# martinber/noaa-apt

Hardware: AMD Instinct MI355X
Metric: Msamples/sec WAV->APT-line decode (higher is better)
Workload: dtype f32; 1 GPU; synthetic 48000 Hz APT recording, 600 s (28800000 samples) per GPU, profile=standard: resample 13/50 (959 taps) -> AM envelope -> 37-tap low-pass -> sync correlation + peak picker -> 1198 rows x 2080 px; parallelism=1 GPU(s), 16 independent recordings per GPU and step, no collectives, recordings_per_call=16, mode=strict, rows=1198, n_sync=1199, input_resident_in_hbm=True, distinct_inputs_round_robin=16

## Files before the change

noaa_apt_amd/csrc/apt_kernels.hpp:

```cpp
#pragma once

#include <hip/hip_runtime.h>

#include <cstdint>

namespace apt::gpu {

struct Result {
    int32_t status;
    int32_t reason;
    uint32_t n_rows;
    uint32_t n_sync;
    uint64_t work_len;
    uint64_t n_out;
};

struct ImageResult {
    int32_t status;
    int32_t reason;
    uint32_t height;
    uint32_t telemetry_row;
    float low, high;
    float telemetry_quality;
    int32_t channel_a, channel_b;
    uint32_t reserved;
    uint64_t n_px;
    float values_a[16], values_b[16];
};

struct GroupMax {
    float hi;
    float lo;
};

struct LaunchSwitches {
    int gather_iters = 1;
    bool words_dpp = true;
    bool orbit_lds = true;
    int orbit_threads = 0;
    int orbit_alg = 1;
    float gm_slack_scale = 1.f;
    int fused_lds_pad = 0;
};
LaunchSwitches read_launch_switches();

constexpr int kMaxCall = 32;
struct RecArgs {
    const void *x;
    uint64_t n;
    uint64_t w;
    float *rows;
    uint32_t rows_cap;
    uint32_t slot;
};
struct CallArgs {
    uint32_t count;
    uint32_t tiles_x;
    RecArgs rec[kMaxCall];
};
struct SlotPtrs {
    float *f;
    GroupMax *gm;
    const float *corr;
    uint64_t *words;
    uint64_t *nanw;
    uint32_t *slot_nt, *slot_cnt, *flags, *orbit_ws, *peaks;
    Result *res;
    uint32_t peaks_cap;
    uint32_t reserved;
};

void resample_generic(hipStream_t s, const float *x, uint64_t n, const float *coeff,
                      uint32_t ntaps, uint32_t l, uint32_t m, float *out, uint64_t w);
uint32_t f16taps_pairs_per_phase(uint32_t l, uint32_t ntaps);
float f16taps_pack(uint32_t l, const float *coeff, uint32_t ntaps, uint16_t *table);
void resample_f16taps(hipStream_t s, const float *x, uint64_t n, const uint16_t *table, uint32_t ntaps,
                      uint32_t l, uint32_t m, float unscale, float *out, uint64_t w);
void fir_decimate(hipStream_t s, const float *x, uint64_t n, const float *coeff, uint32_t ntaps,
                  uint32_t m, float *out, uint64_t n_out);
void demodulate(hipStream_t s, const float *x, uint64_t n, float cosphi2, float sinphi, float *out);
void correlate(hipStream_t s, const float *f, uint64_t n_corr, uint32_t pw, float *corr);
void terminals(hipStream_t s, const float *corr, uint64_t n_corr, uint32_t md, uint64_t *bits);
void orbit_walk(hipStream_t s, const uint64_t *bits, const float *corr, uint64_t n_corr, uint64_t work_len,
                uint32_t spr, uint32_t md, uint32_t *peaks, uint32_t peaks_cap, Result *res);
void gather_rows(hipStream_t s, const float *f, const uint32_t *peaks, Result *res,
                 uint32_t spr, uint32_t pw, bool raw, float *rows, uint32_t rows_cap);
void gather_rows_call(hipStream_t s, const CallArgs &call, const SlotPtrs *d_slots, uint32_t spr, uint32_t pw,
                      uint32_t max_rows_cap, const LaunchSwitches &sw = LaunchSwitches{});

void nosync_rows_call(hipStream_t s, const CallArgs &call, const SlotPtrs *d_slots, uint32_t spr, uint32_t m2, uint64_t max_w);

bool fused_supported(uint32_t l, uint32_t m, uint32_t t1, uint32_t t2, uint32_t pw);
uint32_t fused_group_size(uint32_t l);
bool fused_takes_pcm16(uint32_t l, uint32_t m);
uint32_t fused_tap_table_floats(uint32_t l, uint32_t m, uint32_t t1, int ch);
void fused_branch_taps(uint32_t l, uint32_t m, const float *coeff, uint32_t t1, int ch, float *hs, uint32_t t1_layout = 0);
uint32_t fused_pad_t1(uint32_t l, uint32_t m, uint32_t t1, uint32_t t2, uint32_t pw);
uint32_t fused_pad_t2(uint32_t l, uint32_t m, uint32_t t2, uint32_t pw);
uint32_t fused_phase_pad_t2(uint32_t t2, uint32_t pw);
int fused_chunk_of(uint32_t m, bool fast);
void fused_lowpass_pairs(const float *h2, uint32_t t2, float *h2p);
uint32_t fused_f16_table_dwords(uint32_t l, uint32_t m, uint32_t t1);
float fused_f16_branch_taps(uint32_t l, uint32_t m, const float *coeff, uint32_t t1, uint32_t *table);
bool fused_f16_supported(uint32_t l, uint32_t m, uint32_t t1, uint32_t t2, uint32_t pw);
float fused_gm_slack(uint32_t pw, float scale = 1.f);
bool fused_fast_supported(uint32_t l, uint32_t m, uint32_t t1, uint32_t t2, uint32_t pw);
struct TableGeom {
    uint32_t l, m;
    uint32_t jlim;
    uint32_t tpp;
    uint32_t xt;
    uint32_t off_x;
    uint32_t step_q, step_r;
    uint32_t jl_a, jl_b;
    uint32_t nthr, perm_off, nperm;
    uint32_t nq;
    uint32_t sq;
    uint32_t stream;
    uint32_t exact, perm_shift, cp_off, xd;
    uint32_t tt_off;
// ... 81 lines not shown
```

noaa_apt_amd/csrc/apt_kernels_generic.hip:

```cpp
#include "apt_kernels.hpp"
#include "apt_envelope.hpp"

#include <hip/hip_runtime.h>

#include <cstdlib>

#include <cmath>
#include <cstring>
#include <map>
#include <mutex>
#include <tuple>

#pragma clang fp contract(off)

namespace apt::gpu {

namespace {

constexpr int kBlock = 256;

inline unsigned grid_for(uint64_t n, unsigned block, unsigned cap = 256u * 32u)
{
    uint64_t g = (n + block - 1) / block;
    if (g > cap) g = cap;
// ... 380 lines not shown
    hipLaunchKernelGGL(k_resample_generic, dim3(grid_for(w, kBlock)), dim3(kBlock), 0, s, x, n,
                       coeff, jlim, l, m, out, w);
}

uint32_t f16taps_pairs_per_phase(uint32_t l, uint32_t ntaps) { return ((ntaps + l - 1) / l + 1) / 2; }

float f16taps_pack(uint32_t l, const float *coeff, uint32_t ntaps, uint16_t *table)
{
    const uint32_t jlim = 2 * ((ntaps - 1) / 2) + 1;
    const uint32_t tp2 = f16taps_pairs_per_phase(l, ntaps);
    float mx = 0.f;
    for (uint32_t j = 0; j < jlim; ++j) mx = fmaxf(mx, fabsf(coeff[j]));
    int e = 0;
    if (mx > 0.f) (void)frexpf(mx, &e);
    const int sh = -e + 1;
    const float scale = ldexpf(1.f, sh);
    for (uint32_t p = 0; p < l; ++p)
        for (uint32_t i = 0; i < 2 * tp2; ++i) {
            const uint64_t j = p + static_cast<uint64_t>(i) * l;
            const _Float16 h = static_cast<_Float16>(j < jlim ? coeff[j] * scale : 0.f);
            uint16_t bits;
            __builtin_memcpy(&bits, &h, 2);
            table[(static_cast<size_t>(p) * tp2 * 2) + i] = bits;
        }
    return ldexpf(1.f, -sh);
}

void resample_f16taps(hipStream_t s, const float *x, uint64_t n, const uint16_t *table, uint32_t ntaps,
                      uint32_t l, uint32_t m, float unscale, float *out, uint64_t w)
{
    if (w == 0) return;
    hipLaunchKernelGGL(k_resample_f16taps, dim3(grid_for(w, kBlock)), dim3(kBlock), 0, s, x, n,
                       reinterpret_cast<const h2 *>(table), f16taps_pairs_per_phase(l, ntaps), l, m, unscale,
                       out, w);
}

void fir_decimate(hipStream_t s, const float *x, uint64_t , const float *coeff,
                  uint32_t ntaps, uint32_t m, float *out, uint64_t n_out)
{
    if (n_out == 0) return;
    hipLaunchKernelGGL(k_fir_decimate, dim3(grid_for(n_out, kBlock)), dim3(kBlock), 0, s, x, coeff,
                       ntaps, m, out, n_out);
}

void demodulate(hipStream_t s, const float *x, uint64_t n, float cosphi2, float sinphi, float *out)
{
    if (n == 0) return;
    hipLaunchKernelGGL(k_demodulate, dim3(grid_for(n, kBlock)), dim3(kBlock), 0, s, x, n, cosphi2,
                       sinphi, out);
}

void correlate(hipStream_t s, const float *f, uint64_t n_corr, uint32_t pw, float *corr)
{
    if (n_corr == 0) return;
    hipLaunchKernelGGL(k_correlate, dim3(grid_for(n_corr, kBlock)), dim3(kBlock), 0, s, f, n_corr,
                       pw, corr);
}

void terminals(hipStream_t s, const float *corr, uint64_t n_corr, uint32_t md, uint64_t *bits)
{
    if (n_corr == 0) return;
    const unsigned blocks = static_cast<unsigned>((n_corr + md - 1) / md);
    const size_t lds = static_cast<size_t>(2) * md * sizeof(float);
    if (lds > 48 * 1024)
        (void)hipFuncSetAttribute(reinterpret_cast<const void *>(k_terminals),
                                  hipFuncAttributeMaxDynamicSharedMemorySize,
                                  static_cast<int>(lds));
    hipLaunchKernelGGL(k_terminals, dim3(blocks), dim3(kTermThreads), lds, s, corr, n_corr, md,
                       bits);
}

void orbit_walk(hipStream_t s, const uint64_t *bits, const float *corr, uint64_t n_corr, uint64_t work_len,
                uint32_t spr, uint32_t md, uint32_t *peaks, uint32_t peaks_cap, Result *res)
{
    hipLaunchKernelGGL(k_orbit_walk, dim3(1), dim3(64), 0, s, bits, corr, n_corr, work_len, spr, md,
                       peaks, peaks_cap, res);
}

LaunchSwitches read_launch_switches()
{
    LaunchSwitches sw;
    if (const char *e = std::getenv("APTGPU_GATHER_ITERS")) sw.gather_iters = std::atoi(e);
    if (const char *e = std::getenv("APTGPU_WORDS_DPP")) sw.words_dpp = e[0] != '0';
    if (const char *e = std::getenv("APTGPU_ORBIT_LDS")) sw.orbit_lds = e[0] != '0';
    if (const char *e = std::getenv("APTGPU_ORBIT_THREADS")) sw.orbit_threads = std::atoi(e);
    if (const char *e = std::getenv("APTGPU_ORBIT_ALG")) sw.orbit_alg = e[0] == '0' ? 0 : 1;
    if (const char *e = std::getenv("APTGPU_GM_SLACK_SCALE")) {
        const float v = std::strtof(e, nullptr);
        if (v >= 1.f) sw.gm_slack_scale = v;
    }
    if (const char *e = std::getenv("APTGPU_FUSED_LDS_PAD")) sw.fused_lds_pad = std::max(0, std::atoi(e));
    return sw;
}

void gather_rows_call(hipStream_t s, const CallArgs &call, const SlotPtrs *d_slots, uint32_t spr, uint32_t pw,
                      uint32_t max_rows_cap, const LaunchSwitches &sw)
{
    if (call.count == 0) return;
    {
        const int iters = sw.gather_iters;
        bool aligned = true;
        for (uint32_t i = 0; i < call.count; ++i) aligned = aligned && (reinterpret_cast<uintptr_t>(call.rec[i].rows) & 15u) == 0;
        if (iters > 0 && spr / pw == 2080u && spr % pw == 0 && aligned && max_rows_cap > 0) {
            const uint64_t quads = static_cast<uint64_t>(max_rows_cap < 32768u ? max_rows_cap : 32768u) * 520u;
            const uint64_t per_wg = static_cast<uint64_t>(kBlock) * static_cast<uint64_t>(iters);
            const unsigned gx = static_cast<unsigned>((quads + per_wg - 1) / per_wg);
            hipLaunchKernelGGL(k_gather_rows_flat<520u>, dim3(gx ? gx : 1, call.count), dim3(kBlock), 0, s, call, d_slots, spr, pw);
            return;
        }
    }
    const unsigned rows_cap = max_rows_cap < 32768u ? max_rows_cap : 32768u;
    const unsigned gy = max_rows_cap == 0 ? 1u : (rows_cap + 7u) / 8u;
    const unsigned gx = (spr / pw + 4 * kBlock - 1) / (4 * kBlock);
    hipLaunchKernelGGL(k_gather_rows_call, dim3(gx ? gx : 1, gy, call.count), dim3(kBlock), 0, s, call, d_slots,
                       spr, pw);
}

void gather_rows(hipStream_t s, const float *f, const uint32_t *peaks, Result *res,
                 uint32_t spr, uint32_t pw, bool raw, float *rows, uint32_t rows_cap)
{
    const unsigned gy = rows_cap == 0 ? 1u : (rows_cap < 4096u ? rows_cap : 4096u);
    const unsigned gx = (spr / pw + 4 * kBlock - 1) / (4 * kBlock);
    hipLaunchKernelGGL(k_gather_rows, dim3(gx ? gx : 1, gy), dim3(kBlock), 0, s, f, peaks, res, spr,
                       pw, raw ? 1 : 0, rows, rows_cap);
}


__global__ void __launch_bounds__(256) k_verify_fast_divide(float c, float rc, uint32_t *bad)
{
    const uint32_t i = blockIdx.x * 256u + threadIdx.x;
    const float x = __uint_as_float(0x3F800000u + i);
    const float want = x / c;
    const float got = fast_divide(x, c, rc);
    if (__float_as_uint(want) != __float_as_uint(got)) atomicAdd(bad, 1u);
}

__global__ void __launch_bounds__(256) k_verify_fast_sqrt(uint32_t lo, uint32_t count, uint32_t *bad)
{
    const uint64_t base = (static_cast<uint64_t>(blockIdx.x) * 256u + threadIdx.x) * 64u;
    uint32_t b = 0;
    for (uint32_t i = 0; i < 64u; ++i) {
        const uint64_t idx = base + i;
        if (idx >= count) break;
        const float x = __uint_as_float(lo + static_cast<uint32_t>(idx));
        b += __float_as_uint(exact_sqrt_inrange(x)) != __float_as_uint(__builtin_sqrtf(x));
    }
    if (b) atomicAdd(bad, b);
}

static bool verify_fast_sqrt(int device, hipStream_t s, uint32_t *d_bad)
{
    static std::mutex mu;
    static std::map<int, bool> cache;
    std::lock_guard<std::mutex> lock(mu);
    if (auto it = cache.find(device); it != cache.end()) return it->second;
    constexpr uint32_t lo = 0x0F800000u, hi = 0x71800000u;
    constexpr uint32_t count = hi - lo + 1u, threads = (count + 63u) / 64u;
    uint32_t bad = 1;
    bool ok = hipMemsetAsync(d_bad, 0, sizeof(uint32_t), s) == hipSuccess;
    if (ok) {
        hipLaunchKernelGGL(k_verify_fast_sqrt, dim3((threads + 255u) / 256u), dim3(256), 0, s, lo, count, d_bad);
        ok = hipGetLastError() == hipSuccess &&
             hipMemcpyAsync(&bad, d_bad, sizeof(uint32_t), hipMemcpyDeviceToHost, s) == hipSuccess &&
             hipStreamSynchronize(s) == hipSuccess;
    }
    if (ok) cache[device] = bad == 0;
// ... 39 lines not shown
```

noaa_apt_amd/csrc/apt_kernels_sync.hip:

```cpp
#include "apt_kernels.hpp"
#include "apt_sync_corr.hpp"

#include <hip/hip_runtime.h>

#include <atomic>

#include <cstdlib>
#include <type_traits>

namespace apt::gpu {

namespace {

constexpr int GS = 52;
constexpr uint64_t kGroupMask = (1ull << GS) - 1;
constexpr float kNegInf = -__builtin_huge_valf();

__global__ void __launch_bounds__(256)
k_group_max(const float *__restrict__ corr, uint64_t n_corr, GroupMax *__restrict__ gm, uint32_t ng)
{
    const uint32_t g = blockIdx.x * blockDim.x + threadIdx.x;
    if (g >= ng) return;
    const uint64_t base = static_cast<uint64_t>(g) * GS;
    float mx = kNegInf;
    bool has_nan = false;
    for (int o = 0; o < GS; ++o) {
        const uint64_t i = base + o;
        if (i < n_corr) {
            float v = corr[i];
            if (i == 0 && !(v > 0.f)) v = 0.f;
            mx = fmaxf(mx, v);
            has_nan = has_nan || (v != v);
        }
    }
    gm[g] = has_nan ? GroupMax{-kNegInf, kNegInf} : GroupMax{mx, mx};
}

constexpr int kNodesThreads = 128;
constexpr int kNodesWaves = kNodesThreads / 64;
constexpr int kChunkGroups = 128;
constexpr int kSlotCap = 64;
static_assert(kNodesThreads == kChunkGroups, "one thread per own group");
constexpr uint32_t kNanStartTag = 0x80000000u;
constexpr uint32_t kPosMask = 0x7FFFFFFFu;

__host__ __device__ constexpr uint32_t nodes_window(uint32_t pw) { return (GS + 38u * pw - 1u + 3u) & ~3u; }

__device__ __forceinline__ float wave_prefix_max_dpp(float x)
{
    asm volatile("s_nop 1\n\tv_max_f32_dpp %0, %0, %0 row_shr:1 row_mask:0xf bank_mask:0xf\n\t"
                 "s_nop 1\n\tv_max_f32_dpp %0, %0, %0 row_shr:2 row_mask:0xf bank_mask:0xf\n\t"
                 "s_nop 1\n\tv_max_f32_dpp %0, %0, %0 row_shr:4 row_mask:0xf bank_mask:0xf\n\t"
                 "s_nop 1\n\tv_max_f32_dpp %0, %0, %0 row_shr:8 row_mask:0xf bank_mask:0xf\n\t"
                 "s_nop 1\n\tv_max_f32_dpp %0, %0, %0 row_bcast:15 row_mask:0xa bank_mask:0xf\n\t"
                 "s_nop 1\n\tv_max_f32_dpp %0, %0, %0 row_bcast:31 row_mask:0xc bank_mask:0xf\n\t"
                 "s_nop 1"
                 : "+v"(x));
    return x;
}
__device__ __forceinline__ float wave_suffix_max_excl_dpp(float x, int lane)
{
    float y = -__builtin_huge_valf();
    asm volatile("s_nop 1\n\tv_mov_b32_dpp %0, %1 wave_shl:1 row_mask:0xf bank_mask:0xf\n\t"
                 "s_nop 1\n\tv_max_f32_dpp %0, %0, %0 row_shl:1 row_mask:0xf bank_mask:0xf\n\t"
                 "s_nop 1\n\tv_max_f32_dpp %0, %0, %0 row_shl:2 row_mask:0xf bank_mask:0xf\n\t"
                 "s_nop 1\n\tv_max_f32_dpp %0, %0, %0 row_shl:4 row_mask:0xf bank_mask:0xf\n\t"
                 "s_nop 1\n\tv_max_f32_dpp %0, %0, %0 row_shl:8 row_mask:0xf bank_mask:0xf\n\t"
                 "s_nop 1"
                 : "+v"(y)
                 : "v"(x));
    const float r1 = __builtin_bit_cast(float, __builtin_amdgcn_readlane(__builtin_bit_cast(int, y), 16));
    const float r2 = __builtin_bit_cast(float, __builtin_amdgcn_readlane(__builtin_bit_cast(int, y), 32));
    const float r3 = __builtin_bit_cast(float, __builtin_amdgcn_readlane(__builtin_bit_cast(int, y), 48));
    const float m23 = fmaxf(r2, r3), m123 = fmaxf(r1, m23);
    const float tail = lane < 16 ? m123 : lane < 32 ? m23 : lane < 48 ? r3 : -__builtin_huge_valf();
    return fmaxf(y, tail);
}

__host__ __device__ constexpr uint32_t words_f32_ofs() { return kChunkGroups * 16u; }
__host__ __device__ constexpr uint32_t words_win_ofs(uint32_t r)
{
    return (words_f32_ofs() + (kChunkGroups + r + 1) * 16u + kChunkGroups * 4u + kChunkGroups * 2u + 15u) & ~15u;
}

template <int NL, int PWC>
__device__ __forceinline__ float nodes_eval_window(float *win, bool on, int lane, uint32_t pw, int fast)
{
    constexpr int NLR = NL > 0 ? NL : 1;
    float c = kNegInf;
    if (fast) {
        const uint32_t blen = GS + 36u * pw;
        if constexpr (NL > 0) {
            float bs[NLR];
#pragma unroll
            for (int t = 0; t < NL; ++t) {
                const uint32_t pq = lane + 64u * t;
                bs[t] = pq < blen ? sync_pulse_sum(pw, [&](uint32_t j) { return win[pq + j]; }) : 0.f;
            }
            __builtin_amdgcn_wave_barrier();
#pragma unroll
            for (int t = 0; t < NL; ++t) {
                const uint32_t pq = lane + 64u * t;
                if (pq < blen) win[pq] = bs[t];
            }
            __builtin_amdgcn_wave_barrier();
        } else {
            for (uint32_t p0 = 0; p0 < blen; p0 += 64) {
                const uint32_t pq = p0 + lane;
                const float bs = pq < blen ? sync_pulse_sum(pw, [&](uint32_t j) { return win[pq + j]; }) : 0.f;
                __builtin_amdgcn_wave_barrier();
                if (pq < blen) win[pq] = bs;
                __builtin_amdgcn_wave_barrier();
            }
        }
        if (on) c = sync_corr_from_pulses([&](int k) { return win[lane + k * 2 * pw]; });
    } else {
        if constexpr (PWC >= 4) {
            if (on) c = sync_corr_strict_rolled(pw, [&](uint32_t j) { return win[lane + j]; });
        } else {
            if (on) c = sync_corr_strict(pw, [&](uint32_t j) { return win[lane + j]; });
        }
    }
    return c;
}

template <int NL, int PWC, bool DPP>
__global__ void __launch_bounds__(kNodesThreads, 4)
k_sync_words(const CallArgs call, const SlotPtrs *__restrict__ slots, uint32_t pw_arg, uint32_t r_groups ,
             int fast, int use_corr)
{
    const uint32_t pw = PWC > 0 ? static_cast<uint32_t>(PWC) : pw_arg;
    const RecArgs rec = call.rec[blockIdx.y];
    const uint64_t w = rec.w;
    const uint64_t n_corr = w - 38ull * pw;
    const uint32_t ng = static_cast<uint32_t>((n_corr + GS - 1) / GS);
    if (blockIdx.x * static_cast<uint32_t>(kChunkGroups) >= ng) return;
    const SlotPtrs sp = slots[rec.slot];
    const GroupMax *__restrict__ gm = sp.gm;
    const float *__restrict__ corr = use_corr ? sp.corr : nullptr;
    const float *__restrict__ fsig = sp.f;
    uint32_t *__restrict__ flags = sp.flags;

    extern __shared__ uint64_t lds_nodes[];
    const int R = static_cast<int>(r_groups);
    const int N = kChunkGroups + R + 1;
    uint64_t *s_words = lds_nodes;
    uint64_t *s_nanw = s_words + kChunkGroups;
    float *s_hi = reinterpret_cast<float *>(reinterpret_cast<char *>(lds_nodes) + words_f32_ofs());
    float *s_lo = s_hi + N;
    float *s_ma = s_lo + N;
    float *s_mb = s_ma + N;
    float *s_wm = s_mb + N;
    uint16_t *s_cand = reinterpret_cast<uint16_t *>(s_wm + kChunkGroups);
    const uint32_t wlen = nodes_window(pw);
    float *s_win = reinterpret_cast<float *>(reinterpret_cast<char *>(lds_nodes) + words_win_ofs(r_groups));
    __shared__ uint32_t s_ncand;

    const int tid = threadIdx.x;
    const int lane = tid & 63;
    const int wave = tid >> 6;
    const int64_t g0 = static_cast<int64_t>(blockIdx.x) * kChunkGroups;
    const int64_t gw0 = g0;
    const uint64_t md = static_cast<uint64_t>(R) * GS;

    if (tid == 0) s_ncand = 0;
    if (blockIdx.x == 0 && tid == 0) {
        sp.res->status = -1;
        sp.res->reason = -1;
    }
    for (int q = tid; q < N; q += kNodesThreads) {
        const int64_t g = g0 + q;
        const GroupMax v = g < static_cast<int64_t>(ng) ? gm[g] : GroupMax{kNegInf, kNegInf};
        s_hi[q] = v.hi;
        s_lo[q] = v.lo;
        s_ma[q] = v.lo;
    }
    s_words[tid] = 0ull;
    s_nanw[tid] = 0ull;
    __syncthreads();

    {
        const int W = R - 1;
        float *a = s_ma, *bq = s_mb;
        int K = 1;
        for (; 2 * K <= W; K *= 2) {
            for (int q = tid; q < N; q += kNodesThreads) bq[q] = (q + K < N) ? fmaxf(a[q], a[q + K]) : a[q];
            __syncthreads();
            float *t = a; a = bq; bq = t;
        }
        const int q = tid;
        const int64_t g = g0 + q;
        const float wm = fmaxf(a[q + 1], a[q + 1 + W - K]);
        s_wm[q] = wm;
        if (g < static_cast<int64_t>(ng) && !(wm > s_hi[q])) s_cand[atomicAdd(&s_ncand, 1u)] = static_cast<uint16_t>(q);
        __syncthreads();
    }

    const uint32_t ncand = s_ncand;
    constexpr int kBatch = NL > 0 ? 4 : 1;
    constexpr int NLR = NL > 0 ? NL : 1;
    constexpr uint16_t kDeferred = 0x8000u;
    float *wa = s_win + static_cast<size_t>(wave) * wlen;
    const uint32_t wneed = GS + 38u * pw - 1u;
    auto eval_group = [&](uint64_t base, bool on) -> float {
        for (uint32_t t = lane; t < wlen; t += 64) {
            const uint64_t j = base + t;
            wa[t] = (t < wneed && j < w) ? fsig[j] : 0.f;
        }
        __builtin_amdgcn_wave_barrier();
        const float v = nodes_eval_window<NL, PWC>(wa, on, lane, pw, fast);
        __builtin_amdgcn_wave_barrier();
        return v;
    };
    auto settle = [&](auto exact_tag, int q, float cv, float c2v, bool in_v) -> bool {
        constexpr bool EXACT = decltype(exact_tag)::value;
        const uint64_t base = static_cast<uint64_t>(gw0 + q) * GS;
        const bool in2 = in_v && base + lane + md < n_corr;
        if (in_v && gw0 + q == 0 && lane == 0 && !(cv > 0.f)) cv = 0.f;
        const unsigned long long nanword = __ballot(in_v && cv != cv) & kGroupMask;
        if (cv != cv) cv = kNegInf;
        float sfx_ex;
        if constexpr (DPP) {
            sfx_ex = wave_suffix_max_excl_dpp(cv, lane);
        } else {
            float sfx = cv;
            for (int d = 1; d < 64; d <<= 1) {
                const float o = __shfl_down(sfx, d, 64);
                if (lane + d < 64) sfx = fmaxf(sfx, o);
            }
            sfx_ex = __shfl_down(sfx, 1, 64);
            if (lane == 63) sfx_ex = kNegInf;
        }
        float wm = s_wm[q];
        const bool open_lo = in_v && !(sfx_ex > cv) && !(wm > cv);
        if (__ballot(open_lo) != 0ull) {
            float wm_hi = kNegInf;
            for (int h = q + 1 + lane; h < q + R; h += 64) wm_hi = fmaxf(wm_hi, s_hi[h]);
            for (int d = 32; d >= 1; d >>= 1) wm_hi = fmaxf(wm_hi, __shfl_xor(wm_hi, d, 64));
            const bool open = open_lo && wm_hi > cv;
            if (__ballot(open) != 0ull) {
                if constexpr (!EXACT) {
                    return false;
                } else {
                    float thr = open ? cv : -kNegInf;
                    for (int d = 32; d >= 1; d >>= 1) thr = fminf(thr, __shfl_xor(thr, d, 64));
                    float ex = kNegInf;
#pragma unroll 1
                    for (int h0 = q + 1; h0 < q + R; h0 += 64) {
                        unsigned long long todo = __ballot(h0 + lane < q + R && s_hi[h0 + lane] > thr);
                        while (todo) {
                            const int h = h0 + __ffsll(static_cast<long long>(todo)) - 1;
                            todo &= todo - 1;
                            const int64_t gh = gw0 + h;
                            if (gh >= static_cast<int64_t>(ng)) break;
                            const uint64_t hb = static_cast<uint64_t>(gh) * GS;
                            const bool on = lane < GS && hb + lane < n_corr;
                            float v = kNegInf;
                            if (corr != nullptr) {
                                if (on) v = corr[hb + lane];
                            } else {
                                v = eval_group(hb, on);
                            }
                            if (v != v) v = kNegInf;
                            ex = fmaxf(ex, v);
                        }
                    }
                    for (int d = 32; d >= 1; d >>= 1) ex = fmaxf(ex, __shfl_xor(ex, d, 64));
                    if (open) wm = ex;
                    if (lane == 0) atomicAdd(&flags[7], 1u);
                }
            }
        }
        float wmax = fmaxf(sfx_ex, wm);
        const float gm_ahead = s_hi[q + R];
        if (corr == nullptr && __ballot(in2 && !(wmax > cv) && gm_ahead > cv) != 0ull) c2v = eval_group(base + md, in2);
        if (c2v != c2v) c2v = kNegInf;
        float pfx = c2v;
        if constexpr (DPP) {
            pfx = wave_prefix_max_dpp(pfx);
        } else {
            for (int d = 1; d < 64; d <<= 1) {
                const float o = __shfl_up(pfx, d, 64);
                if (lane >= d) pfx = fmaxf(pfx, o);
            }
        }
        wmax = fmaxf(wmax, pfx);
        const bool term = in_v && !(wmax > cv);
        const unsigned long long word = __ballot(term) & kGroupMask;
        if (lane == 0) {
            s_words[q] = word;
            s_nanw[q] = nanword;
        }
        __builtin_amdgcn_wave_barrier();
        return true;
    };
    bool any_deferred = false;
    for (uint32_t c0 = wave * kBatch; c0 < ncand; c0 += kBatch * kNodesWaves) {
        int qv[kBatch];
        float cv[kBatch], c2v[kBatch];
        bool inv[kBatch];
        float fa[kBatch][NLR];
#pragma unroll
        for (int e = 0; e < kBatch; ++e) {
            const uint32_t ci = c0 + e;
            qv[e] = (ci < ncand) ? s_cand[ci] : -1;
            const int64_t g = gw0 + (qv[e] < 0 ? 0 : qv[e]);
            const uint64_t i = static_cast<uint64_t>(g) * GS + lane;
            inv[e] = qv[e] >= 0 && lane < GS && i < n_corr;
            cv[e] = kNegInf;
            c2v[e] = kNegInf;
            if (corr != nullptr) {
                if (inv[e]) {
                    cv[e] = corr[i];
                    if (i + md < n_corr) c2v[e] = corr[i + md];
                }
            } else if constexpr (NL > 0) {
#pragma unroll
                for (int t = 0; t < NL; ++t) {
                    const uint64_t j = static_cast<uint64_t>(g) * GS + lane + 64u * t;
                    fa[e][t] = (qv[e] >= 0 && lane + 64u * t < wneed && j < w) ? fsig[j] : 0.f;
                }
            }
        }
#pragma unroll
        for (int e = 0; e < kBatch; ++e) {
            if (qv[e] < 0) continue;
            if (corr == nullptr) {
                if constexpr (NL > 0) {
#pragma unroll
                    for (int t = 0; t < NL; ++t)
                        if (lane + 64u * t < wlen) wa[lane + 64 * t] = fa[e][t];
                    __builtin_amdgcn_wave_barrier();
                    cv[e] = nodes_eval_window<NL, PWC>(wa, inv[e], lane, pw, fast);
                    __builtin_amdgcn_wave_barrier();
                } else {
                    cv[e] = eval_group(static_cast<uint64_t>(gw0 + qv[e]) * GS, inv[e]);
                }
            }
            if (!settle(std::false_type{}, qv[e], cv[e], c2v[e], inv[e])) {
                if (lane == 0) s_cand[c0 + e] = static_cast<uint16_t>(qv[e]) | kDeferred;
                any_deferred = true;
            }
        }
    }
    if (any_deferred) {
#pragma unroll 1
        for (uint32_t c0 = wave * kBatch; c0 < ncand; c0 += kBatch * kNodesWaves) {
#pragma unroll 1
            for (uint32_t ci = c0; ci < c0 + kBatch && ci < ncand; ++ci) {
                const uint16_t ent = s_cand[ci];
                if (!(ent & kDeferred)) continue;
                const int q = ent & (kDeferred - 1);
                const uint64_t base = static_cast<uint64_t>(gw0 + q) * GS;
                const bool in_v = lane < GS && base + lane < n_corr;
                float cv = kNegInf, c2v = kNegInf;
                if (corr != nullptr) {
                    if (in_v) {
                        cv = corr[base + lane];
                        if (base + lane + md < n_corr) c2v = corr[base + lane + md];
                    }
                } else {
                    cv = eval_group(base, in_v);
                }
                (void)settle(std::true_type{}, q, cv, c2v, in_v);
            }
        }
    }
    __syncthreads();

    {
        const int64_t g = g0 + tid;
        if (g < static_cast<int64_t>(ng)) {
            sp.words[g] = s_words[tid];
            sp.nanw[g] = s_nanw[tid];
        }
    }
}

__global__ void __launch_bounds__(kNodesThreads)
k_sync_slots(const CallArgs call, const SlotPtrs *__restrict__ slots, uint32_t pw, uint32_t r_groups ,
             uint32_t grid_groups )
{
    const RecArgs rec = call.rec[blockIdx.y];
    const uint64_t n_corr = rec.w - 38ull * pw;
    const uint32_t ng = static_cast<uint32_t>((n_corr + GS - 1) / GS);
    if (blockIdx.x * static_cast<uint32_t>(kChunkGroups) >= ng) return;
    const SlotPtrs sp = slots[rec.slot];
    const uint64_t *__restrict__ words = sp.words;
    const uint64_t *__restrict__ nanw = sp.nanw;
    uint32_t *__restrict__ slot_nt = sp.slot_nt;
    __shared__ uint32_t s_scan[kNodesWaves];
    const int tid = threadIdx.x;
    const int lane = tid & 63;
    const int wave = tid >> 6;
    const int64_t R = r_groups;
    const int64_t g = static_cast<int64_t>(blockIdx.x) * kChunkGroups + tid;
    auto word_at = [&](const uint64_t *p, int64_t gi) -> uint64_t {
        return (gi >= 0 && gi < static_cast<int64_t>(ng)) ? p[gi] : 0ull;
    };
    uint64_t nw = 0, ns = 0;
    if (g < static_cast<int64_t>(ng)) {
        const uint64_t wd = words[g];
        const uint64_t nb = nanw[g];
        const uint64_t prev_bit = word_at(words, g - 1) >> (GS - 1);
        const uint64_t heads = wd & ~(((wd << 1) | prev_bit) & kGroupMask);
        const uint64_t shifted = ((word_at(words, g - R) << 1) | (word_at(words, g - R - 1) >> (GS - 1))) & kGroupMask;
        const uint64_t shifted_nan = ((word_at(nanw, g - R) << 1) | (word_at(nanw, g - R - 1) >> (GS - 1))) & kGroupMask;
        const uint64_t on_grid = (g % grid_groups == 0) ? 1ull : 0ull;
        const uint64_t starts = shifted | shifted_nan | on_grid;
        nw = wd & (heads | starts);
        ns = nb & starts & ~wd;
    }
    const uint32_t cnt = static_cast<uint32_t>(__popcll(nw | ns));
    uint32_t inc = cnt;
    for (int d = 1; d < 64; d <<= 1) {
        const uint32_t o = __shfl_up(inc, d, 64);
        if (lane >= d) inc += o;
    }
    if (lane == 63) s_scan[wave] = inc;
    __syncthreads();
    uint32_t base = 0;
    for (int wv = 0; wv < wave; ++wv) base += s_scan[wv];
    uint32_t total = 0;
    for (int wv = 0; wv < kNodesWaves; ++wv) total += s_scan[wv];
    uint32_t ofs = base + inc - cnt;
    uint64_t bitsleft = nw | ns;
    while (bitsleft) {
        const int bpos = __ffsll(static_cast<long long>(bitsleft)) - 1;
        bitsleft &= bitsleft - 1;
        if (ofs < kSlotCap)
            slot_nt[static_cast<uint64_t>(blockIdx.x) * kSlotCap + ofs] =
                static_cast<uint32_t>(static_cast<uint64_t>(g) * GS + bpos) | (((ns >> bpos) & 1ull) ? kNanStartTag : 0u);
        ++ofs;
    }
    if (tid == 0) {
        sp.slot_cnt[blockIdx.x] = total;
        if (total > kSlotCap) atomicOr(&sp.flags[0], 1u);
    }
}

constexpr int kOrbitThreadsMax = 1024;
constexpr int kMaxLevels = 64;

struct OrbitGeom {
    uint64_t n_corr, work_len;
    uint32_t spr, md;
};

__device__ __forceinline__ uint64_t first_terminal52(const uint64_t *__restrict__ words,
                                                     uint64_t n_groups, uint64_t s)
{
    const int lane = threadIdx.x & 63;
    uint64_t g0 = s / GS;
    const uint32_t sh = static_cast<uint32_t>(s % GS);
    bool first = true;
    while (true) {
        const uint64_t gi = g0 + lane;
        uint64_t word = (gi < n_groups) ? words[gi] : 0ull;
        if (first && lane == 0) word &= (~0ull) << sh;
        const unsigned long long any = __ballot(word != 0ull);
        if (any) {
            const int src = __ffsll(static_cast<long long>(any)) - 1;
            const uint64_t pos = gi * GS + (__ffsll(static_cast<long long>(word)) - 1);
            return __shfl(pos, src, 64);
        }
        first = false;
        g0 += 64;
        if (g0 >= n_groups) return ~0ull;
    }
}

__device__ void orbit_walk52(const uint64_t *__restrict__ words, const uint64_t *__restrict__ nanw,
                             const OrbitGeom &gq, uint32_t *__restrict__ peaks, uint32_t peaks_cap,
                             Result *__restrict__ res)
{
    auto nan_at = [&](uint64_t s) -> bool { return (nanw[s / GS] >> (s % GS)) & 1ull; };
    const int lane = threadIdx.x & 63;
    const uint64_t n_groups = (gq.n_corr + GS - 1) / GS;
    const uint64_t spr = gq.spr, md = gq.md;
    uint64_t len = 1;
    uint64_t u = 0;
    if (gq.n_corr > 0) u = first_terminal52(words, n_groups, 0);
    if (lane == 0 && peaks_cap > 0) peaks[0] = static_cast<uint32_t>(u);
    uint64_t fit = (u + spr < gq.work_len) ? 1 : 0;
    uint64_t last_fit = fit;
    while (gq.n_corr > 0) {
        const uint64_t a = u + md + 1;
        const uint64_t b = (len + 1) * spr;
        const uint64_t s = a > b ? a : b;
        if (s >= gq.n_corr) break;
        const uint64_t c = s / spr;
        for (uint64_t q = len + lane; q + 1 < c; q += 64)
            if (q < peaks_cap) peaks[q] = static_cast<uint32_t>(s);
        if (s + spr < gq.work_len) fit += c - len - 1;
        u = nan_at(s) ? s : first_terminal52(words, n_groups, s);
        if (lane == 0 && c - 1 < peaks_cap) peaks[c - 1] = static_cast<uint32_t>(u);
        last_fit = (u + spr < gq.work_len) ? 1 : 0;
        fit += last_fit;
        len = c;
    }
// ... 614 lines not shown
    }
    unsigned long long fit_local = 0;
    for (uint32_t k = tid; !peaks_done && k < path_cap; k += NT) {
        const uint32_t v = gld(w_path + k);
        if (v == END) continue;
        uint32_t cell;
        const uint32_t sv = node_start(v, &cell);
        const uint32_t u = gld(w_u + v);
        const bool is_last = (k + 1 >= path_cap) || gld(w_path + k + 1) == END;
        if (k == 0) {
            if (peaks_cap > 0) peaks[0] = u;
            if (!is_last && u + spr < wl32) ++fit_local;
            if (is_last) s_plen = 1;
            continue;
        }
        uint32_t pcell;
        (void)node_start(gld(w_path + k - 1), &pcell);
        const uint32_t c_prev = (k - 1 == 0) ? 1u : pcell;
        const uint32_t c = cell;
        for (uint32_t qv = c_prev; qv + 1 < c; ++qv)
            if (qv < peaks_cap) peaks[qv] = sv;
        if (c - 1 < peaks_cap) peaks[c - 1] = u;
        if (sv + spr < wl32) fit_local += c - c_prev - 1;
        if (!is_last && u + spr < wl32) ++fit_local;
        if (is_last) s_plen = c;
    }
    if (!peaks_done) {
    {
        uint32_t f32v = static_cast<uint32_t>(fit_local);
        for (int d = 32; d >= 1; d >>= 1) f32v += __shfl_down(f32v, d, 64);
        if ((tid & 63) == 0 && f32v) atomicAdd(&s_fit, static_cast<unsigned long long>(f32v));
    }
    __syncthreads();
    }
    if (tid == 0) {
        const uint32_t len = s_plen;
        const bool few = len < 5;
        const uint64_t rows = s_fit;
        res->status = few ? 1 : 0;
        res->reason = few ? 2 : 0;
        res->n_sync = len;
        res->n_rows = few ? 0 : static_cast<uint32_t>(rows);
        res->work_len = gq.work_len;
        res->n_out = few ? 0 : rows * 2080u;
        flags[1] = 2u;
        flags[0] = 0u;
        flags[5] = 0u;
        flags[2] = nt_cap;
        flags[3] = n_nodes;
        flags[4] = all_done ? n_all : count;
        flags[6] = all_done ? 3u : direct ? 1u : (in_lds ? 2u : 0u);
        if (all_done) flags[12] = 0u;
        flags[11] = flags7;
        flags[7] = 0u;
    }
    stamp(2);
}

}

uint32_t sync_group_size() { return GS; }
uint32_t sync_chunk_groups() { return kChunkGroups; }
uint32_t sync_slot_cap() { return kSlotCap; }

void group_max(hipStream_t s, const float *corr, uint64_t n_corr, GroupMax *gm)
{
    const uint32_t ng = static_cast<uint32_t>((n_corr + GS - 1) / GS);
    if (ng == 0) return;
    hipLaunchKernelGGL(k_group_max, dim3((ng + 255) / 256), dim3(256), 0, s, corr, n_corr, gm, ng);
}

void sync_nodes(hipStream_t s, const CallArgs &call, const SlotPtrs *d_slots, uint64_t max_w, uint32_t pw,
                uint32_t spr, uint32_t md, bool fast, bool use_corr, const LaunchSwitches &sw)
{
    if (call.count == 0 || max_w <= 38ull * pw) return;
    const uint64_t n_corr = max_w - 38ull * pw;
    const uint32_t ng = static_cast<uint32_t>((n_corr + GS - 1) / GS);
    const uint32_t chunks = (ng + kChunkGroups - 1) / kChunkGroups;
    const uint32_t r = md / GS;
    const size_t lds = words_win_ofs(r) + static_cast<size_t>(kNodesWaves) * nodes_window(pw) * sizeof(float);
    const dim3 grid(chunks, call.count);
    const uint32_t wneed = GS + 38u * pw - 1u;
    const bool dpp = sw.words_dpp;
#define APT_WORDS_LAUNCH(NL, PWC)                                                                                       \
    do {                                                                                                                \
        if (dpp)                                                                                                        \
            hipLaunchKernelGGL((k_sync_words<NL, PWC, true>), grid, dim3(kNodesThreads), lds, s, call, d_slots, pw, r,  \
                               fast ? 1 : 0, use_corr ? 1 : 0);                                                         \
        else                                                                                                            \
            hipLaunchKernelGGL((k_sync_words<NL, PWC, false>), grid, dim3(kNodesThreads), lds, s, call, d_slots, pw, r, \
                               fast ? 1 : 0, use_corr ? 1 : 0);                                                         \
    } while (0)
    if (pw == 3) APT_WORDS_LAUNCH(3, 3);
    else if (pw == 4) APT_WORDS_LAUNCH(4, 4);
    else if (pw == 5) APT_WORDS_LAUNCH(4, 5);
    else if (wneed <= 192) APT_WORDS_LAUNCH(3, 0);
    else if (wneed <= 256) APT_WORDS_LAUNCH(4, 0);
    else APT_WORDS_LAUNCH(0, 0);
#undef APT_WORDS_LAUNCH
    hipLaunchKernelGGL(k_sync_slots, grid, dim3(kNodesThreads), 0, s, call, d_slots, pw, r, spr / GS);
}

uint32_t sync_nt_cap(uint64_t w)
{
    const uint64_t ng = (w + GS - 1) / GS;
    const uint64_t chunks = (ng + kChunkGroups - 1) / kChunkGroups;
    return static_cast<uint32_t>(chunks * kSlotCap);
}

size_t sync_orbit_ws_words(uint64_t w, uint32_t spr)
{
    const uint64_t nt_cap = sync_nt_cap(w);
    const uint64_t kc = (spr ? w / spr : 0) + 2;
    const uint64_t node_cap = 1 + kc + nt_cap + 1;
    return 4 * node_cap + (node_cap / 32 + 1) + (kc + 2) + (kc + 3) + 64;
}

static bool orbit_all_nodes_available(uint32_t bytes)
{
    constexpr int kMaxDevices = 64;
    static std::atomic<int> state[kMaxDevices];
    int dev = 0;
    (void)hipGetDevice(&dev);
    if (dev < 0 || dev >= kMaxDevices) dev = 0;
    int st = state[dev].load(std::memory_order_acquire);
    if (st == 0) {
        int max_lds = 0;
        const bool ok = hipDeviceGetAttribute(&max_lds, hipDeviceAttributeMaxSharedMemoryPerBlock, dev) == hipSuccess &&
                        max_lds >= static_cast<int>(bytes) &&
                        hipFuncSetAttribute(reinterpret_cast<const void *>(&k_sync_orbit_global<kOrbitThreadsMax>),
                                            hipFuncAttributeMaxDynamicSharedMemorySize, static_cast<int>(bytes)) == hipSuccess;
        (void)hipGetLastError();
        st = ok ? 1 : 2;
        state[dev].store(st, std::memory_order_release);
    }
    return st == 1;
}

void sync_orbit(hipStream_t s, const CallArgs &call, const SlotPtrs *d_slots, uint32_t spr, uint32_t md,
                uint32_t pw, int force, const LaunchSwitches &sw)
{
    if (call.count == 0) return;
    const uint32_t kOrbitLdsEntries = sw.orbit_lds ? 12288u : 0u;
    constexpr uint32_t kAllEntries = 65536u;
    const int alg = (sw.orbit_alg == 0 || kOrbitLdsEntries == 0u || !orbit_all_nodes_available(kAllEntries * sizeof(uint16_t))) ? 0 : 1;
    if (sw.orbit_threads == 256) {
        hipLaunchKernelGGL(k_sync_orbit_global<256>, dim3(call.count), dim3(256), kOrbitLdsEntries * sizeof(uint16_t), s,
                           call, d_slots, spr, md, pw, force == 1 ? 1 : 0, kOrbitLdsEntries, 0);
    } else if (alg == 1) {
        hipLaunchKernelGGL(k_sync_orbit_global<kOrbitThreadsMax>, dim3(call.count), dim3(kOrbitThreadsMax), kAllEntries * sizeof(uint16_t), s,
                           call, d_slots, spr, md, pw, force == 1 ? 1 : 0, kAllEntries, 1);
    } else {
        hipLaunchKernelGGL(k_sync_orbit_global<kOrbitThreadsMax>, dim3(call.count), dim3(kOrbitThreadsMax), kOrbitLdsEntries * sizeof(uint16_t), s,
                           call, d_slots, spr, md, pw, force == 1 ? 1 : 0, kOrbitLdsEntries, 0);
    }
}

}
```

Baseline: 550,600 Msamples/s.

## Add lean sync-words form with block prefix/suffix window max and interior fast paths

```diff
diff --git a/noaa_apt_amd/csrc/apt_kernels.hpp b/noaa_apt_amd/csrc/apt_kernels.hpp
--- a/noaa_apt_amd/csrc/apt_kernels.hpp
+++ b/noaa_apt_amd/csrc/apt_kernels.hpp
@@ -36,6 +36,7 @@
 struct LaunchSwitches {
     int gather_iters = 1;
     bool words_dpp = true;
+    int words_form = 1;
     bool orbit_lds = true;
     int orbit_threads = 0;
     int orbit_alg = 1;
diff --git a/noaa_apt_amd/csrc/apt_kernels_generic.hip b/noaa_apt_amd/csrc/apt_kernels_generic.hip
--- a/noaa_apt_amd/csrc/apt_kernels_generic.hip
+++ b/noaa_apt_amd/csrc/apt_kernels_generic.hip
@@ -486,6 +486,7 @@
     LaunchSwitches sw;
     if (const char *e = std::getenv("APTGPU_GATHER_ITERS")) sw.gather_iters = std::atoi(e);
     if (const char *e = std::getenv("APTGPU_WORDS_DPP")) sw.words_dpp = e[0] != '0';
+    if (const char *e = std::getenv("APTGPU_WORDS_FORM")) sw.words_form = e[0] == '0' ? 0 : 1;
     if (const char *e = std::getenv("APTGPU_ORBIT_LDS")) sw.orbit_lds = e[0] != '0';
     if (const char *e = std::getenv("APTGPU_ORBIT_THREADS")) sw.orbit_threads = std::atoi(e);
     if (const char *e = std::getenv("APTGPU_ORBIT_ALG")) sw.orbit_alg = e[0] == '0' ? 0 : 1;
diff --git a/noaa_apt_amd/csrc/apt_kernels_sync.hip b/noaa_apt_amd/csrc/apt_kernels_sync.hip
--- a/noaa_apt_amd/csrc/apt_kernels_sync.hip
+++ b/noaa_apt_amd/csrc/apt_kernels_sync.hip
@@ -13,6 +13,12 @@
 namespace {
 
 constexpr int GS = 52;
+
+#ifdef APT_WORDS_MARKS
+#define APT_WMARK(what) asm volatile("; APTMARK " what)
+#else
+#define APT_WMARK(what) ((void)0)
+#endif
 constexpr uint64_t kGroupMask = (1ull << GS) - 1;
 constexpr float kNegInf = -__builtin_huge_valf();
 
@@ -77,6 +83,12 @@
     return fmaxf(y, tail);
 }
 
+__device__ __forceinline__ float wave_max_all_dpp(float x)
+{
+    x = wave_prefix_max_dpp(x);
+    return __builtin_bit_cast(float, __builtin_amdgcn_readlane(__builtin_bit_cast(int, x), 63));
+}
+
 __host__ __device__ constexpr uint32_t words_f32_ofs() { return kChunkGroups * 16u; }
 __host__ __device__ constexpr uint32_t words_win_ofs(uint32_t r)
 {
@@ -124,7 +136,7 @@
     return c;
 }
 
-template <int NL, int PWC, bool DPP>
+template <int NL, int PWC, bool DPP, bool LEAN>
 __global__ void __launch_bounds__(kNodesThreads, 4)
 k_sync_words(const CallArgs call, const SlotPtrs *__restrict__ slots, uint32_t pw_arg, uint32_t r_groups ,
              int fast, int use_corr)
@@ -168,54 +180,98 @@
         sp.res->status = -1;
         sp.res->reason = -1;
     }
-    for (int q = tid; q < N; q += kNodesThreads) {
-        const int64_t g = g0 + q;
-        const GroupMax v = g < static_cast<int64_t>(ng) ? gm[g] : GroupMax{kNegInf, kNegInf};
-        s_hi[q] = v.hi;
-        s_lo[q] = v.lo;
-        s_ma[q] = v.lo;
-    }
-    s_words[tid] = 0ull;
-    s_nanw[tid] = 0ull;
-    __syncthreads();
-
-    {
-        const int W = R - 1;
-        float *a = s_ma, *bq = s_mb;
-        int K = 1;
-        for (; 2 * K <= W; K *= 2) {
-            for (int q = tid; q < N; q += kNodesThreads) bq[q] = (q + K < N) ? fmaxf(a[q], a[q + K]) : a[q];
+    APT_WMARK("BEGIN coarse");
+    static_assert(!LEAN || (DPP && NL > 0 && PWC > 0), "the lean form builds on the DPP scans and the register-held windows");
+    if constexpr (LEAN) {
+        constexpr int RC = 32 * PWC, NC = kChunkGroups + RC + 1, NB = (NC + 63) / 64;
+        static_assert(RC - 2 >= 64 && 2 * NB * 64 <= 3 * NC, "a window spans two blocks or more; P and S fit");
+        float *s_p = s_lo, *s_s = s_lo + NB * 64;
+        const GroupMax *__restrict__ gmb = gm + g0;
+        const uint32_t n_left = ng - static_cast<uint32_t>(g0);
+#pragma unroll
+        for (int k = 0; k < (NB + kNodesWaves - 1) / kNodesWaves; ++k) {
+            const int b = wave + k * kNodesWaves;
+            if (b < NB) {
+                const uint32_t q = b * 64u + lane, qr = b * 64u + 63u - lane;
+                const GroupMax v = (q < NC && q < n_left) ? gmb[q] : GroupMax{kNegInf, kNegInf};
+                const float lo_r = (qr < NC && qr < n_left) ? gmb[qr].lo : kNegInf;
+                if (q < NC) s_hi[q] = v.hi;
+                s_p[q] = wave_prefix_max_dpp(v.lo);
+                s_s[qr] = wave_prefix_max_dpp(lo_r);
+            }
+        }
+        s_words[tid] = 0ull;
+        s_nanw[tid] = 0ull;
+        __syncthreads();
+        const int q = tid;
+        const int a = q + 1, e = q + RC - 1;
+        float wm = fmaxf(s_s[a], s_p[e]);
+#pragma unroll
+        for (int b = 1; b < NB - 1; ++b) {
+            const float whole = s_s[b * 64];
+            wm = (b > (a >> 6) && b < (e >> 6)) ? fmaxf(wm, whole) : wm;
+        }
+        s_wm[q] = wm;
+        if (static_cast<uint32_t>(q) < n_left && !(wm > s_hi[q])) s_cand[atomicAdd(&s_ncand, 1u)] = static_cast<uint16_t>(q);
+        __syncthreads();
+    } else {
+        for (int q = tid; q < N; q += kNodesThreads) {
+            const int64_t g = g0 + q;
+            const GroupMax v = g < static_cast<int64_t>(ng) ? gm[g] : GroupMax{kNegInf, kNegInf};
+            s_hi[q] = v.hi;
+            s_lo[q] = v.lo;
+            s_ma[q] = v.lo;
+        }
+        s_words[tid] = 0ull;
+        s_nanw[tid] = 0ull;
+        __syncthreads();
+
+        {
+            const int W = R - 1;
+            float *a = s_ma, *bq = s_mb;
+            int K = 1;
+            for (; 2 * K <= W; K *= 2) {
+                for (int q = tid; q < N; q += kNodesThreads) bq[q] = (q + K < N) ? fmaxf(a[q], a[q + K]) : a[q];
+                __syncthreads();
+                float *t = a; a = bq; bq = t;
+            }
+            const int q = tid;
+            const int64_t g = g0 + q;
+            const float wm = fmaxf(a[q + 1], a[q + 1 + W - K]);
+            s_wm[q] = wm;
+            if (g < static_cast<int64_t>(ng) && !(wm > s_hi[q])) s_cand[atomicAdd(&s_ncand, 1u)] = static_cast<uint16_t>(q);
             __syncthreads();
-            float *t = a; a = bq; bq = t;
-        }
-        const int q = tid;
-        const int64_t g = g0 + q;
-        const float wm = fmaxf(a[q + 1], a[q + 1 + W - K]);
-        s_wm[q] = wm;
-        if (g < static_cast<int64_t>(ng) && !(wm > s_hi[q])) s_cand[atomicAdd(&s_ncand, 1u)] = static_cast<uint16_t>(q);
-        __syncthreads();
-    }
-
+        }
+    }
+
+    APT_WMARK("END coarse");
     const uint32_t ncand = s_ncand;
     constexpr int kBatch = NL > 0 ? 4 : 1;
     constexpr int NLR = NL > 0 ? NL : 1;
     constexpr uint16_t kDeferred = 0x8000u;
     float *wa = s_win + static_cast<size_t>(wave) * wlen;
     const uint32_t wneed = GS + 38u * pw - 1u;
-    auto eval_group = [&](uint64_t base, bool on) -> float {
-        for (uint32_t t = lane; t < wlen; t += 64) {
-            const uint64_t j = base + t;
-            wa[t] = (t < wneed && j < w) ? fsig[j] : 0.f;
+    auto eval_group = [&](auto int_tag, uint64_t base, bool on) -> float {
+        if constexpr (decltype(int_tag)::value) {
+            const float *__restrict__ fb = fsig + base;
+            for (uint32_t t = lane; t < wlen; t += 64) wa[t] = fb[t];
+        } else {
+            for (uint32_t t = lane; t < wlen; t += 64) {
+                const uint64_t j = base + t;
+                wa[t] = (t < wneed && j < w) ? fsig[j] : 0.f;
+            }
         }
         __builtin_amdgcn_wave_barrier();
         const float v = nodes_eval_window<NL, PWC>(wa, on, lane, pw, fast);
         __builtin_amdgcn_wave_barrier();
         return v;
     };
-    auto settle = [&](auto exact_tag, int q, float cv, float c2v, bool in_v) -> bool {
+    auto settle = [&](auto exact_tag, auto int_tag, int q, float cv, float c2v, bool in_v) -> bool {
         constexpr bool EXACT = decltype(exact_tag)::value;
+        constexpr bool INT = decltype(int_tag)::value;
+        APT_WMARK("BEGIN settle");
         const uint64_t base = static_cast<uint64_t>(gw0 + q) * GS;
-        const bool in2 = in_v && base + lane + md < n_corr;
+        const bool in2 = INT ? in_v : (in_v && base + lane + md < n_corr);
         if (in_v && gw0 + q == 0 && lane == 0 && !(cv > 0.f)) cv = 0.f;
         const unsigned long long nanword = __ballot(in_v && cv != cv) & kGroupMask;
         if (cv != cv) cv = kNegInf;
@@ -236,14 +292,22 @@
         if (__ballot(open_lo) != 0ull) {
             float wm_hi = kNegInf;
             for (int h = q + 1 + lane; h < q + R; h += 64) wm_hi = fmaxf(wm_hi, s_hi[h]);
-            for (int d = 32; d >= 1; d >>= 1) wm_hi = fmaxf(wm_hi, __shfl_xor(wm_hi, d, 64));
+            if constexpr (LEAN) {
+                wm_hi = wave_max_all_dpp(wm_hi);
+            } else {
+                for (int d = 32; d >= 1; d >>= 1) wm_hi = fmaxf(wm_hi, __shfl_xor(wm_hi, d, 64));
+            }
             const bool open = open_lo && wm_hi > cv;
             if (__ballot(open) != 0ull) {
                 if constexpr (!EXACT) {
                     return false;
                 } else {
                     float thr = open ? cv : -kNegInf;
-                    for (int d = 32; d >= 1; d >>= 1) thr = fminf(thr, __shfl_xor(thr, d, 64));
+                    if constexpr (LEAN) {
+                        thr = -wave_max_all_dpp(-thr);
+                    } else {
+                        for (int d = 32; d >= 1; d >>= 1) thr = fminf(thr, __shfl_xor(thr, d, 64));
+                    }
                     float ex = kNegInf;
 #pragma unroll 1
                     for (int h0 = q + 1; h0 < q + R; h0 += 64) {
@@ -254,18 +318,22 @@
                             const int64_t gh = gw0 + h;
                             if (gh >= static_cast<int64_t>(ng)) break;
                             const uint64_t hb = static_cast<uint64_t>(gh) * GS;
-                            const bool on = lane < GS && hb + lane < n_corr;
+                            const bool on = lane < GS && (INT || hb + lane < n_corr);
                             float v = kNegInf;
                             if (corr != nullptr) {
                                 if (on) v = corr[hb + lane];
                             } else {
-                                v = eval_group(hb, on);
+                                v = eval_group(int_tag, hb, on);
                             }
                             if (v != v) v = kNegInf;
                             ex = fmaxf(ex, v);
                         }
                     }
-                    for (int d = 32; d >= 1; d >>= 1) ex = fmaxf(ex, __shfl_xor(ex, d, 64));
+                    if constexpr (LEAN) {
+                        ex = wave_max_all_dpp(ex);
+                    } else {
+                        for (int d = 32; d >= 1; d >>= 1) ex = fmaxf(ex, __shfl_xor(ex, d, 64));
+                    }
                     if (open) wm = ex;
                     if (lane == 0) atomicAdd(&flags[7], 1u);
                 }
@@ -273,7 +341,7 @@
         }
         float wmax = fmaxf(sfx_ex, wm);
         const float gm_ahead = s_hi[q + R];
-        if (corr == nullptr && __ballot(in2 && !(wmax > cv) && gm_ahead > cv) != 0ull) c2v = eval_group(base + md, in2);
+        if (corr == nullptr && __ballot(in2 && !(wmax > cv) && gm_ahead > cv) != 0ull) c2v = eval_group(int_tag, base + md, in2);
         if (c2v != c2v) c2v = kNegInf;
         float pfx = c2v;
         if constexpr (DPP) {
@@ -292,82 +360,107 @@
             s_nanw[q] = nanword;
         }
         __builtin_amdgcn_wave_barrier();
+        APT_WMARK("END settle");
         return true;
     };
-    bool any_deferred = false;
-    for (uint32_t c0 = wave * kBatch; c0 < ncand; c0 += kBatch * kNodesWaves) {
-        int qv[kBatch];
-        float cv[kBatch], c2v[kBatch];
-        bool inv[kBatch];
-        float fa[kBatch][NLR];
-#pragma unroll
-        for (int e = 0; e < kBatch; ++e) {
-            const uint32_t ci = c0 + e;
-            qv[e] = (ci < ncand) ? s_cand[ci] : -1;
-            const int64_t g = gw0 + (qv[e] < 0 ? 0 : qv[e]);
-            const uint64_t i = static_cast<uint64_t>(g) * GS + lane;
-            inv[e] = qv[e] >= 0 && lane < GS && i < n_corr;
-            cv[e] = kNegInf;
-            c2v[e] = kNegInf;
-            if (corr != nullptr) {
-                if (inv[e]) {
-                    cv[e] = corr[i];
-                    if (i + md < n_corr) c2v[e] = corr[i + md];
-                }
-            } else if constexpr (NL > 0) {
-#pragma unroll
-                for (int t = 0; t < NL; ++t) {
-                    const uint64_t j = static_cast<uint64_t>(g) * GS + lane + 64u * t;
-                    fa[e][t] = (qv[e] >= 0 && lane + 64u * t < wneed && j < w) ? fsig[j] : 0.f;
-                }
-            }
-        }
-#pragma unroll
-        for (int e = 0; e < kBatch; ++e) {
-            if (qv[e] < 0) continue;
-            if (corr == nullptr) {
-                if constexpr (NL > 0) {
-#pragma unroll
-                    for (int t = 0; t < NL; ++t)
-                        if (lane + 64u * t < wlen) wa[lane + 64 * t] = fa[e][t];
-                    __builtin_amdgcn_wave_barrier();
-                    cv[e] = nodes_eval_window<NL, PWC>(wa, inv[e], lane, pw, fast);
-                    __builtin_amdgcn_wave_barrier();
-                } else {
-                    cv[e] = eval_group(static_cast<uint64_t>(gw0 + qv[e]) * GS, inv[e]);
-                }
-            }
-            if (!settle(std::false_type{}, qv[e], cv[e], c2v[e], inv[e])) {
-                if (lane == 0) s_cand[c0 + e] = static_cast<uint16_t>(qv[e]) | kDeferred;
-                any_deferred = true;
-            }
-        }
-    }
-    if (any_deferred) {
+    const uint32_t per_wave = (ncand + kNodesWaves - 1) / kNodesWaves;
+    const uint32_t c_lo = LEAN ? wave * per_wave : wave * kBatch;
+    const uint32_t c_hi = LEAN ? (c_lo + per_wave < ncand ? c_lo + per_wave : ncand) : ncand;
+    const uint32_t c_step = LEAN ? kBatch : kBatch * kNodesWaves;
+    auto fine_passes = [&](auto int_tag) {
+        constexpr bool INT = decltype(int_tag)::value;
+        bool any_deferred = false;
+        for (uint32_t c0 = c_lo; c0 < c_hi; c0 += c_step) {
+            int qv[kBatch];
+            float cv[kBatch], c2v[kBatch];
+            bool inv[kBatch];
+            float fa[kBatch][NLR];
+            APT_WMARK("BEGIN window-load");
+#pragma unroll
+            for (int e = 0; e < kBatch; ++e) {
+                const uint32_t ci = c0 + e;
+                qv[e] = (ci < c_hi) ? s_cand[ci] : -1;
+                if constexpr (LEAN) qv[e] = __builtin_amdgcn_readfirstlane(qv[e]);
+                const int64_t g = gw0 + (qv[e] < 0 ? 0 : qv[e]);
+                const uint64_t i = static_cast<uint64_t>(g) * GS + lane;
+                inv[e] = qv[e] >= 0 && lane < GS && (INT || i < n_corr);
+                cv[e] = kNegInf;
+                c2v[e] = kNegInf;
+                if constexpr (INT) {
+                    const float *__restrict__ fb = fsig + static_cast<uint64_t>(g) * GS;
+#pragma unroll
+                    for (int t = 0; t < NL; ++t) fa[e][t] = fb[static_cast<uint32_t>(lane) + 64u * t];
+                } else if (corr != nullptr) {
+                    if (inv[e]) {
+                        cv[e] = corr[i];
+                        if (i + md < n_corr) c2v[e] = corr[i + md];
+                    }
+                } else if constexpr (NL > 0) {
+#pragma unroll
+                    for (int t = 0; t < NL; ++t) {
+                        const uint64_t j = static_cast<uint64_t>(g) * GS + lane + 64u * t;
+                        fa[e][t] = (qv[e] >= 0 && lane + 64u * t < wneed && j < w) ? fsig[j] : 0.f;
+                    }
+                }
+            }
+            APT_WMARK("END window-load");
+#pragma unroll
+            for (int e = 0; e < kBatch; ++e) {
+                if (qv[e] < 0) continue;
+                APT_WMARK("BEGIN stage+chain");
+                if (corr == nullptr) {
+                    if constexpr (NL > 0) {
+#pragma unroll
+                        for (int t = 0; t < NL; ++t)
+                            if (lane + 64u * t < wlen) wa[lane + 64 * t] = fa[e][t];
+                        __builtin_amdgcn_wave_barrier();
+                        cv[e] = nodes_eval_window<NL, PWC>(wa, inv[e], lane, pw, fast);
+                        __builtin_amdgcn_wave_barrier();
+                    } else {
+                        cv[e] = eval_group(int_tag, static_cast<uint64_t>(gw0 + qv[e]) * GS, inv[e]);
+                    }
+                }
+                APT_WMARK("END stage+chain");
+                if (!settle(std::false_type{}, int_tag, qv[e], cv[e], c2v[e], inv[e])) {
+                    if (lane == 0) s_cand[c0 + e] = static_cast<uint16_t>(qv[e]) | kDeferred;
+                    any_deferred = true;
+                }
+            }
+        }
+        if (any_deferred) {
 #pragma unroll 1
-        for (uint32_t c0 = wave * kBatch; c0 < ncand; c0 += kBatch * kNodesWaves) {
+            for (uint32_t c0 = c_lo; c0 < c_hi; c0 += c_step) {
 #pragma unroll 1
-            for (uint32_t ci = c0; ci < c0 + kBatch && ci < ncand; ++ci) {
-                const uint16_t ent = s_cand[ci];
-                if (!(ent & kDeferred)) continue;
-                const int q = ent & (kDeferred - 1);
-                const uint64_t base = static_cast<uint64_t>(gw0 + q) * GS;
-                const bool in_v = lane < GS && base + lane < n_corr;
-                float cv = kNegInf, c2v = kNegInf;
-                if (corr != nullptr) {
-                    if (in_v) {
-                        cv = corr[base + lane];
-                        if (base + lane + md < n_corr) c2v = corr[base + lane + md];
-                    }
-                } else {
-                    cv = eval_group(base, in_v);
-                }
-                (void)settle(std::true_type{}, q, cv, c2v, in_v);
-            }
-        }
+                for (uint32_t ci = c0; ci < c0 + kBatch && ci < c_hi; ++ci) {
+                    const uint16_t ent = s_cand[ci];
+                    if (!(ent & kDeferred)) continue;
+                    int q = ent & (kDeferred - 1);
+                    if constexpr (LEAN) q = __builtin_amdgcn_readfirstlane(q);
+                    const uint64_t base = static_cast<uint64_t>(gw0 + q) * GS;
+                    const bool in_v = lane < GS && (INT || base + lane < n_corr);
+                    float cv = kNegInf, c2v = kNegInf;
+                    if (corr != nullptr) {
+                        if (in_v) {
+                            cv = corr[base + lane];
+                            if (base + lane + md < n_corr) c2v = corr[base + lane + md];
+                        }
+                    } else {
+                        cv = eval_group(int_tag, base, in_v);
+                    }
+                    (void)settle(std::true_type{}, int_tag, q, cv, c2v, in_v);
+                }
+            }
+        }
+    };
+    if (LEAN && corr == nullptr &&
+        static_cast<uint64_t>(g0 + kChunkGroups + R + 1) * GS <= n_corr) {
+        if constexpr (LEAN) fine_passes(std::true_type{});
+    } else {
+        fine_passes(std::false_type{});
     }
     __syncthreads();
 
+    APT_WMARK("BEGIN write-out");
     {
         const int64_t g = g0 + tid;
         if (g < static_cast<int64_t>(ng)) {
@@ -375,8 +468,10 @@
             sp.nanw[g] = s_nanw[tid];
         }
     }
-}
-
+    APT_WMARK("END write-out");
+}
+
+template <bool SKIP>
 __global__ void __launch_bounds__(kNodesThreads)
 k_sync_slots(const CallArgs call, const SlotPtrs *__restrict__ slots, uint32_t pw, uint32_t r_groups ,
              uint32_t grid_groups )
@@ -399,9 +494,11 @@
         return (gi >= 0 && gi < static_cast<int64_t>(ng)) ? p[gi] : 0ull;
     };
     uint64_t nw = 0, ns = 0;
-    if (g < static_cast<int64_t>(ng)) {
-        const uint64_t wd = words[g];
-        const uint64_t nb = nanw[g];
+    const bool own = g < static_cast<int64_t>(ng);
+    const uint64_t wd = own ? words[g] : 0ull;
+    const uint64_t nb = own ? nanw[g] : 0ull;
+    const bool busy = !SKIP || __ballot((wd | nb) != 0ull) != 0ull;
+    if (own && busy) {
         const uint64_t prev_bit = word_at(words, g - 1) >> (GS - 1);
         const uint64_t heads = wd & ~(((wd << 1) | prev_bit) & kGroupMask);
         const uint64_t shifted = ((word_at(words, g - R) << 1) | (word_at(words, g - R - 1) >> (GS - 1))) & kGroupMask;
@@ -413,9 +510,11 @@
     }
     const uint32_t cnt = static_cast<uint32_t>(__popcll(nw | ns));
     uint32_t inc = cnt;
-    for (int d = 1; d < 64; d <<= 1) {
-        const uint32_t o = __shfl_up(inc, d, 64);
-        if (lane >= d) inc += o;
+    if (busy) {
+        for (int d = 1; d < 64; d <<= 1) {
+            const uint32_t o = __shfl_up(inc, d, 64);
+            if (lane >= d) inc += o;
+        }
     }
     if (lane == 63) s_scan[wave] = inc;
     __syncthreads();
@@ -1196,23 +1295,37 @@
     const dim3 grid(chunks, call.count);
     const uint32_t wneed = GS + 38u * pw - 1u;
     const bool dpp = sw.words_dpp;
+    const bool lean = sw.words_form != 0 && dpp && r == 32u * pw;
+#define APT_WORDS_LAUNCH_(NL, PWC, DPP, LEAN)                                                                           \
+    hipLaunchKernelGGL((k_sync_words<NL, PWC, DPP, LEAN>), grid, dim3(kNodesThreads), lds, s, call, d_slots, pw, r,     \
+                       fast ? 1 : 0, use_corr ? 1 : 0)
 #define APT_WORDS_LAUNCH(NL, PWC)                                                                                       \
     do {                                                                                                                \
         if (dpp)                                                                                                        \
-            hipLaunchKernelGGL((k_sync_words<NL, PWC, true>), grid, dim3(kNodesThreads), lds, s, call, d_slots, pw, r,  \
-                               fast ? 1 : 0, use_corr ? 1 : 0);                                                         \
+            APT_WORDS_LAUNCH_(NL, PWC, true, false);                                                                    \
         else                                                                                                            \
-            hipLaunchKernelGGL((k_sync_words<NL, PWC, false>), grid, dim3(kNodesThreads), lds, s, call, d_slots, pw, r, \
-                               fast ? 1 : 0, use_corr ? 1 : 0);                                                         \
+            APT_WORDS_LAUNCH_(NL, PWC, false, false);                                                                   \
     } while (0)
-    if (pw == 3) APT_WORDS_LAUNCH(3, 3);
-    else if (pw == 4) APT_WORDS_LAUNCH(4, 4);
-    else if (pw == 5) APT_WORDS_LAUNCH(4, 5);
+#define APT_WORDS_LAUNCH_PW(NL, PWC)                                                                                    \
+    do {                                                                                                                \
+        if (lean)                                                                                                       \
+            APT_WORDS_LAUNCH_(NL, PWC, true, true);                                                                     \
+        else                                                                                                            \
+            APT_WORDS_LAUNCH(NL, PWC);                                                                                  \
+    } while (0)
+    if (pw == 3) APT_WORDS_LAUNCH_PW(3, 3);
+    else if (pw == 4) APT_WORDS_LAUNCH_PW(4, 4);
+    else if (pw == 5) APT_WORDS_LAUNCH_PW(4, 5);
     else if (wneed <= 192) APT_WORDS_LAUNCH(3, 0);
     else if (wneed <= 256) APT_WORDS_LAUNCH(4, 0);
     else APT_WORDS_LAUNCH(0, 0);
+#undef APT_WORDS_LAUNCH_PW
 #undef APT_WORDS_LAUNCH
-    hipLaunchKernelGGL(k_sync_slots, grid, dim3(kNodesThreads), 0, s, call, d_slots, pw, r, spr / GS);
+#undef APT_WORDS_LAUNCH_
+    if (sw.words_form != 0)
+        hipLaunchKernelGGL(k_sync_slots<true>, grid, dim3(kNodesThreads), 0, s, call, d_slots, pw, r, spr / GS);
+    else
+        hipLaunchKernelGGL(k_sync_slots<false>, grid, dim3(kNodesThreads), 0, s, call, d_slots, pw, r, spr / GS);
 }
 
 uint32_t sync_nt_cap(uint64_t w)
```

Result: faster. 565,200 Msamples/s, median of 6 (+2.7%).
